# Ighina/MultimodalTopicSegmentation

Measured on AMD Instinct MI355X. Metric: sentences/sec (fwd+bwd), higher is better.
Workload: dtype bf16; 1 GPU; BASELINE configs[1]: restricted-window transformer tagger d=1792 heads=8 ff=256 radius=15 layers=1 focal loss, 64 docs x 256 sentences per GPU, fwd+bwd+Adam(eps 1e-7), inputs resident in HBM; global_batch_docs=64, sentences_per_doc=256, parallelism=dp1 (document-sharded, RCCL all-reduce)

## Files before the change

multimodaltopicsegmentation_amd/csrc/gemm.hip:

```cpp
#include <algorithm>
#include <math.h>
#include <stdlib.h>
#include "common.h"

#include "gemm_common.h"


template <int LAYOUT, typename TC, bool GLDS>
__global__ __launch_bounds__(256, 2) void gemm_bf16_kernel(const GemmArgs a) {
  constexpr bool A_KMAJOR = (LAYOUT == MTS_NT || LAYOUT == MTS_NN);
  constexpr bool B_KMAJOR = (LAYOUT == MTS_NT || LAYOUT == MTS_TT);
  extern __shared__ __attribute__((aligned(16))) char smem[];

  const int tid = threadIdx.x;
  const int lane = tid & 63;
  const int wave = tid >> 6;
  const int wm = wave >> 1, wn = wave & 1;
  const int r16 = lane & 15, g = lane >> 4;

  const int ntn = (a.N + BN - 1) / BN;
  const int ntm = (a.M + BM - 1) / BM;
  const int nt = ntn * ntm;
  int bid = xcd_remap(blockIdx.x, nt);
  const int bm0 = (ntm < ntn ? bid % ntm : bid / ntn) * BM;
// ... 549 lines not shown
    const int e = (int)(i - r * q) * 4;
    float v[4];
    load4<float>(e < D1 ? s1 + r * D1 + e : s2 + r * D2 + (e - D1), v);
    store4<T>(dst + r * D + e, v);
  }
}

extern "C" int mts_cast_concat(void* stream, int dst_dtype, size_t rows, int D1, int D2, const float* src1, const float* src2, void* dst) {
  MTS_CHECK_ARG(src1 && src2 && dst && D1 > 0 && D2 > 0 && D1 % 4 == 0 && D2 % 4 == 0, "mts_cast_concat: bad arguments (widths must be multiples of 4)");
  if (rows == 0) return MTS_OK;
  const int blocks = (int)std::min<size_t>(4096, (rows * ((D1 + D2) / 4) + 255) / 256);
  if (dst_dtype == MTS_BF16) hipLaunchKernelGGL(cast_concat_kernel<bf16_t>, dim3(blocks), dim3(256), 0, (hipStream_t)stream, src1, src2, (bf16_t*)dst, rows, D1, D2);
  else if (dst_dtype == MTS_F32) hipLaunchKernelGGL(cast_concat_kernel<float>, dim3(blocks), dim3(256), 0, (hipStream_t)stream, src1, src2, (float*)dst, rows, D1, D2);
  else { mts_set_error("mts_cast_concat: bad dtype %d", dst_dtype); return MTS_ERR_INVALID; }
  MTS_LAUNCH_CHECK("mts_cast_concat");
  return MTS_OK;
}

extern "C" size_t mts_colsum_workspace(int N) { return (size_t)COLSUM_RS * (size_t)N * sizeof(float); }

extern "C" int mts_colsum(void* stream, int dtype, int M, int N, const void* X, int ldx, float* out, int accumulate,
                          void* partial) {
  MTS_CHECK_ARG(M > 0 && N > 0 && X && out && partial, "mts_colsum: bad arguments");
  MTS_CHECK_ARG(dtype == MTS_F32 || dtype == MTS_BF16, "mts_colsum: bad dtype %d", dtype);
  MTS_CHECK_ARG(ldx % 4 == 0, "mts_colsum: ldx must be a multiple of 4");
  hipStream_t st = (hipStream_t)stream;
  const int nparts = min(COLSUM_RS, M);
  dim3 grid(ceil_div(N, 64), COLSUM_RS);
  (void)nparts;
  if (dtype == MTS_F32)
    hipLaunchKernelGGL(colsum_partial_kernel<float>, grid, dim3(256), 0, st, (const float*)X, M, N, ldx, (float*)partial);
  else
    hipLaunchKernelGGL(colsum_partial_kernel<bf16_t>, grid, dim3(256), 0, st, (const bf16_t*)X, M, N, ldx, (float*)partial);
  hipLaunchKernelGGL(colsum_final_kernel, dim3(ceil_div(N, 64)), dim3(256), 0, st, (const float*)partial, N, COLSUM_RS, out,
                     accumulate);
  MTS_LAUNCH_CHECK("mts_colsum");
  return MTS_OK;
}

extern "C" int mts_cast(void* stream, int dst_dtype, const float* src, void* dst, size_t n) {
  MTS_CHECK_ARG(src && dst, "mts_cast: null pointer");
  if (n == 0) return MTS_OK;
  hipStream_t st = (hipStream_t)stream;
  const int blocks = (int)std::min<size_t>(2048, (n / 4 + 255) / 256 + 1);
  if (dst_dtype == MTS_BF16)
    hipLaunchKernelGGL(cast_kernel<bf16_t>, dim3(blocks), dim3(256), 0, st, src, (bf16_t*)dst, n);
  else if (dst_dtype == MTS_F32)
    hipLaunchKernelGGL(cast_kernel<float>, dim3(blocks), dim3(256), 0, st, src, (float*)dst, n);
  else {
    mts_set_error("mts_cast: bad dtype %d", dst_dtype);
    return MTS_ERR_INVALID;
  }
  MTS_LAUNCH_CHECK("mts_cast");
  return MTS_OK;
}

int mts_launch_gemm256(const GemmArgs& a, int layout, bool c_is_f32, int splits, hipStream_t st);
int mts_launch_gemm224(const GemmArgs& a, int layout, bool c_is_f32, int splits, hipStream_t st);
bool mts_gemm224t_applies(const GemmArgs& a, int layout, bool c_is_f32, int splits);

static thread_local int g_gemm_glds = -1;
static thread_local int g_tile_mode = -1;
static thread_local int g_force_splits = 0;
static thread_local int g_tile_order = 1;
static thread_local int g_gemm_deep = 1;
static thread_local int g_chain = 0;
static thread_local int g_combine = 0;
#define MTS_GEMM_WS_HEAD 8192
static thread_local int g_last_tile = 0, g_last_splits = 0;

static thread_local void (*g_mid_hook)(void) = nullptr;
extern "C" int mts_gemm_set_mid_hook(void (*fn)(void)) { g_mid_hook = fn; return MTS_OK; }

extern "C" int mts_gemm_last_plan(int* tile, int* splits) {
  if (tile) *tile = g_last_tile;
  if (splits) *splits = g_last_splits;
  return MTS_OK;
}

void mts_band_set_mfma(int on);
void mts_band_set_fused(int on);
void mts_full_set_mfma(int on);
void mts_t5_set_mfma(int on);
static thread_local int g_f32_mfma = 1;
static thread_local int g_big_min_k = 256;
static thread_local int g_gemm_variant = 0;
void mts_lstm_pair_set_spin_limit(int n);
void mts_lstm_pair_set_max_pairs(int n);
void mts_lstm_pair_set_parts(int n);
extern "C" int mts_set_option(const char* key, int value) {
  if (!key) return MTS_ERR_INVALID;
  if (!strcmp(key, "gemm_tile")) { g_tile_mode = value; return MTS_OK; }
  if (!strcmp(key, "gemm_glds")) { g_gemm_glds = value; return MTS_OK; }
  if (!strcmp(key, "gemm_splits")) { g_force_splits = value; return MTS_OK; }
  if (!strcmp(key, "gemm_order")) { g_tile_order = value; return MTS_OK; }
  if (!strcmp(key, "gemm_chain")) { g_chain = value; return MTS_OK; }
  if (!strcmp(key, "gemm_combine")) { g_combine = value; return MTS_OK; }
  if (!strcmp(key, "gemm_deep")) { g_gemm_deep = value; return MTS_OK; }
  if (!strcmp(key, "gemm_variant")) { g_gemm_variant = value; return MTS_OK; }
  if (!strcmp(key, "gemm_big_min_k")) { g_big_min_k = value; return MTS_OK; }
  if (!strcmp(key, "gemm_f32_mfma")) { g_f32_mfma = value; return MTS_OK; }
  if (!strcmp(key, "band_mfma")) { mts_band_set_mfma(value); return MTS_OK; }
  if (!strcmp(key, "band_fused_bwd")) { mts_band_set_fused(value); return MTS_OK; }
  if (!strcmp(key, "full_mfma")) { mts_full_set_mfma(value); return MTS_OK; }
  if (!strcmp(key, "t5_mfma")) { mts_t5_set_mfma(value); return MTS_OK; }
  if (!strcmp(key, "lstm_pair_spin_limit")) { mts_lstm_pair_set_spin_limit(value); return MTS_OK; }
  if (!strcmp(key, "lstm_pair_max_pairs")) { mts_lstm_pair_set_max_pairs(value); return MTS_OK; }
  if (!strcmp(key, "lstm_parts")) { mts_lstm_pair_set_parts(value); return MTS_OK; }
  mts_set_error("mts_set_option: unknown key %s", key);
  return MTS_ERR_INVALID;
}

template <int LAYOUT, typename TC>
static void launch_bf16(const GemmArgs& a, int splits, hipStream_t st) {
  const int nt = ceil_div(a.M, BM) * ceil_div(a.N, BN);
  if (g_gemm_glds < 0) {
    const char* e = getenv("MTS_GEMM_GLDS");
    g_gemm_glds = (e && e[0] == '0') ? 0 : 1;
  }
  const bool glds = g_gemm_glds && (a.K % BK == 0) && (a.ksplit % BK == 0) && a.M >= 8 && a.N >= 8;
  if (glds) {
    GemmArgs b = a;
    const bool deep = g_gemm_deep && (size_t)nt * splits <= 256 && a.ksplit >= 4 * BK;
    b.nbuf = deep ? 4 : 2;
    auto k = gemm_bf16_kernel<LAYOUT, TC, true>;
    if (deep && mts_dyn_lds(k, 8 * TILE_BYTES, "gemm") != MTS_OK) b.nbuf = 2;
    hipLaunchKernelGGL(k, dim3(nt, 1, splits), dim3(256), (b.nbuf == 4 ? 8 : 4) * TILE_BYTES, st, b);
  } else {
    hipLaunchKernelGGL((gemm_bf16_kernel<LAYOUT, TC, false>), dim3(nt, 1, splits), dim3(256), 4 * TILE_BYTES, st, a);
  }
}

static void plan_bf16(int c_dtype, int layout, int M, int N, int K, unsigned epilogue, bool has_workspace, size_t workspace_bytes,
                      int* use256_out, int* splits_out) {
  if (g_tile_mode < 0) {
    const char* e = getenv("MTS_GEMM_TILE");
    g_tile_mode = e ? atoi(e) : 0;
  }
  const int tile_mode = g_tile_mode;
  const unsigned plain = epilogue & ~MTS_EPI_ACCUM;
  const bool can_split = (c_dtype == MTS_F32 && plain == 0 && has_workspace && N % 4 == 0 && K >= 2048);
  const bool can256 = (K % BK == 0) && K >= g_big_min_k && M >= 8 && N >= 8 && tile_mode != 128;
  const double bw = 3500.0;
  double best = 1e30;
  int splits = 1;
  int use256 = 0;
  const bool can224 = can256 && (N % 224 == 0) && tile_mode != 256;
  for (int big = 0; big <= (can256 ? 2 : 0); ++big) {
    if (big == 2 && !can224) continue;
    if (tile_mode == 256 && can256 && big != 1) continue;
    if (tile_mode == 224 && can224 && big != 2) continue;
    const int tile = big ? 256 : 128;
    const double slots = big ? 256.0 : 512.0;
    const double t_k = layout == MTS_TN ? (big == 2 ? (M % 256 == 0 ? 0.0160 : 0.0200) : big == 1 ? 0.0218 : 0.0145)
                                        : (big ? 0.0232 * (big == 2 ? 0.875 : 1.0) : 0.0180);
    const double t_0 = big ? 7.7 : 6.5;
    const int nt = ceil_div(M, tile) * (big == 2 ? N / 224 : ceil_div(N, tile));
    for (int sp = 1; sp <= (can_split ? 32 : 1); ++sp) {
      const int ks = ceil_div(ceil_div(K, sp), BK) * BK;
      if (ceil_div(K, ks) != sp) continue;
      if (sp > 1 && (size_t)sp * M * N * sizeof(float) > workspace_bytes) break;
      if (g_force_splits > 0 && can_split && sp != g_force_splits) continue;
      const double rounds = ceil((double)nt * sp / slots);
      const double cost = rounds * (ks * t_k + t_0) + (sp > 1 ? (2.0 * sp + 1.0) * M * N * 4.0 / 1e6 / bw : 0.0);
      if (cost < best) { best = cost; splits = sp; use256 = big; }
    }
  }
  *use256_out = use256;
  *splits_out = splits;
}

int mts_gemm224_last_kernel();
int mts_launch_gemm224t_pair(const GemmArgs& a, int splits, const void* A2, const void* B2, float* slab2, hipStream_t st);
bool mts_gemm224t_applies(const GemmArgs& a, int layout, bool c_is_f32, int splits);

static int wgrad_pair_splits(int M, int N, int K, size_t workspace_bytes) {
  if (M % 256 || N % 224 || K % 64 || K < 256) return -1;
  static int cus = 0;
  if (!cus) { int dev = 0; hipDeviceProp_t pr; cus = (hipGetDevice(&dev) == hipSuccess && hipGetDeviceProperties(&pr, dev) == hipSuccess) ? pr.multiProcessorCount : 256; }
  const int nt = (M / 256) * (N / 224);
  int sp = std::max(1, std::min(32, cus / (2 * nt)));
  for (; sp >= 1; --sp) {
    const int ks = ceil_div(ceil_div(K, sp), BK) * BK;
    if (ceil_div(K, ks) != sp) continue;
    if (ks >= 128 && K - (sp - 1) * ks >= 128 && (size_t)2 * sp * M * N * sizeof(float) <= workspace_bytes) return sp;
  }
  return -1;
}
// ... 158 lines not shown
```

multimodaltopicsegmentation_amd/csrc/norm.hip:

```cpp
#include <algorithm>
#include <type_traits>
#include "common.h"
#include "loss_elems.h"

#define ROW_WAVES 4
#define BWD_MAX_BLOCKS 512

template <typename T, int NV> struct RowRegs {
  float v[NV][4];
  __device__ __forceinline__ void load(const T* row, int D, int lane) {
#pragma unroll
    for (int i = 0; i < NV; ++i) {
      const int e = 4 * (lane + 64 * i);
      if (e < D) load4<T>(row + e, v[i]);
      else { v[i][0] = v[i][1] = v[i][2] = v[i][3] = 0.f; }
    }
  }
  __device__ __forceinline__ void store(T* row, int D, int lane) const {
#pragma unroll
    for (int i = 0; i < NV; ++i) {
      const int e = 4 * (lane + 64 * i);
      if (e < D) store4<T>(row + e, v[i]);
    }
  }
  __device__ __forceinline__ void zero() {
#pragma unroll
    for (int i = 0; i < NV; ++i) v[i][0] = v[i][1] = v[i][2] = v[i][3] = 0.f;
  }
};

template <int NV> __device__ __forceinline__ void row_stats(const float (&x)[NV][4], int D, int lane, float& mean, float& rstd, float eps) {
  float s = 0.f;
#pragma unroll
  for (int i = 0; i < NV; ++i) s += (x[i][0] + x[i][1]) + (x[i][2] + x[i][3]);
  mean = wave_sum(s) / (float)D;
  float q = 0.f;
#pragma unroll
  for (int i = 0; i < NV; ++i) {
    if (4 * (lane + 64 * i) < D) {
#pragma unroll
      for (int j = 0; j < 4; ++j) { const float d = x[i][j] - mean; q += d * d; }
    }
  }
  rstd = 1.0f / sqrtf(wave_sum(q) / (float)D + eps);
}

template <typename T, int NV, int EMBED, bool FULL = false>
__global__ __launch_bounds__(64 * ROW_WAVES) void ln_fwd_kernel(
    const void* __restrict__ xin, const float* __restrict__ pos, int pos_offset, int L, const float* __restrict__ type0,
    const float* __restrict__ gamma, const float* __restrict__ beta, float eps, int rows, int D,
    T* __restrict__ y, T* __restrict__ pre, float* __restrict__ mean_out, float* __restrict__ rstd_out,
    const float* __restrict__ head_w, const float* __restrict__ head_b, int n_out, float* __restrict__ scores,
    const int32_t* __restrict__ row_src, const float* __restrict__ xin2 = nullptr, int D1 = 0) {
  const int lane = threadIdx.x & 63;
  const int row = blockIdx.x * ROW_WAVES + (threadIdx.x >> 6);
  if (row >= rows) return;
  float gv[NV][4], bv[NV][4];
#pragma unroll
  for (int i = 0; i < NV; ++i) {
    const int e = 4 * (lane + 64 * i);
    if (FULL || e < D) { load4<float>(gamma + e, gv[i]); load4<float>(beta + e, bv[i]); }
  }
  float x[NV][4];
  if constexpr (EMBED) {
    const int src = row_src ? row_src[row] : row;
    const int Dx = xin2 ? D1 : D;
    const float* xr = reinterpret_cast<const float*>(xin) + (size_t)src * Dx;
    const float* xr2 = xin2 ? xin2 + (size_t)src * (D - D1) - D1 : xr;
    const float* pr = pos + (size_t)(pos_offset + src % L) * D;
#pragma unroll
    for (int i = 0; i < NV; ++i) {
      const int e = 4 * (lane + 64 * i);
      if (FULL || e < D) {
        float a[4], b[4], c[4];
        if constexpr (EMBED == 2) load4<bf16_t>(reinterpret_cast<const bf16_t*>(xin) + (size_t)src * D + e, a);
        else load4<float>((e < Dx ? xr : xr2) + e, a);
        load4<float>(pr + e, b); load4<float>(type0 + e, c);
#pragma unroll
        for (int j = 0; j < 4; ++j) x[i][j] = (a[j] + b[j]) + c[j];
        if constexpr (sizeof(T) == 2) {
#pragma unroll
          for (int j = 0; j < 4; ++j) x[i][j] = to_f32(from_f32<T>(x[i][j]));
        }
      } else { x[i][0] = x[i][1] = x[i][2] = x[i][3] = 0.f; }
    }
    if (pre) {
#pragma unroll
      for (int i = 0; i < NV; ++i) { const int e = 4 * (lane + 64 * i); if (FULL || e < D) store4<T>(pre + (size_t)row * D + e, x[i]); }
    }
  } else {
    const T* xr = reinterpret_cast<const T*>(xin) + (size_t)row * D;
#pragma unroll
    for (int i = 0; i < NV; ++i) {
      const int e = 4 * (lane + 64 * i);
      if (FULL || e < D) load4<T>(xr + e, x[i]);
      else { x[i][0] = x[i][1] = x[i][2] = x[i][3] = 0.f; }
    }
  }
  float mean, rstd;
  row_stats<NV>(x, D, lane, mean, rstd, eps);
  float hs[4] = {0.f, 0.f, 0.f, 0.f};
  const float* hwp = head_w ? head_w : gamma;
  const int hw_max = head_w ? n_out - 1 : 0;
#pragma unroll
  for (int i = 0; i < NV; ++i) {
    const int e = 4 * (lane + 64 * i);
    if (FULL || e < D) {
#pragma unroll
      for (int j = 0; j < 4; ++j) x[i][j] = (x[i][j] - mean) * rstd * gv[i][j] + bv[i][j];
      if (head_w) {
#pragma unroll
        for (int c = 0; c < 4; ++c) {
          float w[4];
          load4<float>(hwp + (size_t)min(c, hw_max) * D + e, w);
#pragma unroll
          for (int j = 0; j < 4; ++j) hs[c] += to_f32(from_f32<T>(x[i][j])) * w[j];
        }
      }
    }
  }
  if (y) {
#pragma unroll
    for (int i = 0; i < NV; ++i) {
      const int e = 4 * (lane + 64 * i);
      if (FULL || e < D) store4<T>(y + (size_t)row * D + e, x[i]);
    }
  }
  if (lane == 0 && mean_out) { mean_out[row] = mean; rstd_out[row] = rstd; }
  if (head_w) {
    for (int c = 0; c < n_out; ++c) {
      const float s = wave_sum(hs[c]);
      if (lane == 0) scores[(size_t)row * n_out + c] = s + head_b[c];
    }
  }
}

template <typename T>
__global__ __launch_bounds__(64 * ROW_WAVES) void head_fwd_kernel(const T* __restrict__ x, int ldx, int rows, int D, int n_out,
                                                                const float* __restrict__ w, const float* __restrict__ b,
                                                                float* __restrict__ scores) {
  const int lane = threadIdx.x & 63;
  const int row = blockIdx.x * ROW_WAVES + (threadIdx.x >> 6);
  if (row >= rows) return;
  float hs[4] = {0.f, 0.f, 0.f, 0.f};
  for (int e = 4 * lane; e < D; e += 256) {
    float xv[4];
    load4<T>(x + (size_t)row * ldx + e, xv);
    for (int c = 0; c < n_out; ++c) {
      float wv[4];
      load4<float>(w + (size_t)c * D + e, wv);
#pragma unroll
      for (int j = 0; j < 4; ++j) hs[c] += xv[j] * wv[j];
    }
  }
  for (int c = 0; c < n_out; ++c) {
    const float s = wave_sum(hs[c]);
    if (lane == 0) scores[(size_t)row * n_out + c] = s + b[c];
  }
}

template <typename T>
__global__ __launch_bounds__(256) void head_bwd_data_kernel(const float* __restrict__ ds, const float* __restrict__ w, int rows, int D,
                                                            int n_out, T* __restrict__ dx, int lddx, int accumulate) {
  const size_t idx = (size_t)blockIdx.x * 256 + threadIdx.x;
  const int per_row = D / 4;
  const size_t total = (size_t)rows * per_row;
  if (idx >= total) return;
  const int row = (int)(idx / per_row);
  const int e = 4 * (int)(idx % per_row);
  float o[4] = {0.f, 0.f, 0.f, 0.f};
  if (accumulate) load4<T>(dx + (size_t)row * lddx + e, o);
  for (int c = 0; c < n_out; ++c) {
    const float s = ds[(size_t)row * n_out + c];
    float wv[4];
    load4<float>(w + (size_t)c * D + e, wv);
#pragma unroll
    for (int j = 0; j < 4; ++j) o[j] += s * wv[j];
  }
  store4<T>(dx + (size_t)row * lddx + e, o);
}

struct EmbArgs { int B, L, Bc, nchunks; const int32_t* row0; const int32_t* lengths; float* dpos_part; };

template <typename T, int NV, bool WIDE, bool FULL = false, int NHG = 0, bool EMB = false>
__global__ __launch_bounds__(64 * ROW_WAVES, 2) void ln_bwd_kernel(
    const T* __restrict__ x, const T* __restrict__ dy_, const float* __restrict__ dlogit, const float* __restrict__ head_w, int n_out,
    const float* __restrict__ gamma, const float* __restrict__ mean, const float* __restrict__ rstd, int rows, int D,
    T* __restrict__ dx, float* __restrict__ partial, const EmbArgs ea) {
  static_assert(!(EMB && (WIDE || NHG > 0)), "the embedding form has no head and D <= 2048");
  constexpr bool HG = NHG > 0;
  constexpr int NR = HG ? NHG + 1 : EMB ? 2 : 3;
  constexpr int NS = HG ? NHG + 2 : NR;
  constexpr int NA = HG ? NHG : 2;
  const T* __restrict__ dy = HG ? nullptr : dy_;
  __shared__ float red[ROW_WAVES][NR][64 * 4];
  __shared__ __attribute__((aligned(16))) float gam_s[NV * 256];
  __shared__ __attribute__((aligned(16))) float hw_s[EMB ? 1 : 4][EMB ? 4 : NV * 256];
  __shared__ __attribute__((aligned(16))) float task_s[EMB ? ROW_WAVES : 1][EMB ? NV * 256 : 4];
  const int lane = threadIdx.x & 63;
  const int wave = __builtin_amdgcn_readfirstlane(threadIdx.x >> 6);
  const int col0 = WIDE ? (int)blockIdx.y * (NV * 256) : 0;
  for (int idx = threadIdx.x; idx < NV * 256; idx += 64 * ROW_WAVES) {
    const int e = col0 + idx;
    gam_s[idx] = (e < D) ? gamma[e] : 0.f;
    if constexpr (!EMB) {
      if (head_w)
        for (int c = 0; c < n_out; ++c) hw_s[c][idx] = (e < D) ? head_w[(size_t)c * D + e] : 0.f;
    }
  }
  __syncthreads();
  float acc[NA][NV][4];
  float dxs[NV][4];
  float tsum[HG ? NHG : 1];
#pragma unroll
  for (int i = 0; i < NV; ++i)
#pragma unroll
    for (int j = 0; j < 4; ++j) {
// ... 685 lines not shown
    else { const float tv[4] = {t.x, t.y, t.z, t.w}; for (int j = 0; j < 4 && e + j < len; ++j) o[e + j] = tv[j]; }
  }
}

int mts_slab_reduce_rows(hipStream_t st, const float* partial, int nblocks, int D, float* out) {
  SlabOuts so = {{out, nullptr, nullptr, nullptr, nullptr, nullptr}, -1, 0, nullptr, -1, 0};
  hipLaunchKernelGGL(slab_reduce_kernel, dim3(ceil_div(D, SR_COLS), 1), dim3(256), 0, st, partial, nblocks, 1, D, so);
  MTS_LAUNCH_CHECK("slab_reduce");
  return MTS_OK;
}

template <typename T>
__global__ __launch_bounds__(256) void embed_bwd_kernel(const T* __restrict__ dpre, int B, int L, int D, float* __restrict__ dpos, int pos_offset,
                                                        const int32_t* __restrict__ row0, const int32_t* __restrict__ lengths) {
  const size_t idx = (size_t)blockIdx.x * 256 + threadIdx.x;
  const int per_row = D / 4;
  if (idx >= (size_t)L * per_row) return;
  const int i = (int)(idx / per_row), e = 4 * (int)(idx % per_row);
  float s[4] = {0.f, 0.f, 0.f, 0.f};
  int b = 0;
  if (row0) {
    for (; b < B; ++b) {
      if (i < lengths[b]) {
        float v[4];
        load4<T>(dpre + ((size_t)row0[b] + i) * D + e, v);
#pragma unroll
        for (int j = 0; j < 4; ++j) s[j] += v[j];
      }
    }
  }
  for (; b + 7 < B; b += 8) {
    float v[8][4];
#pragma unroll
    for (int u = 0; u < 8; ++u) load4<T>(dpre + ((size_t)(b + u) * L + i) * D + e, v[u]);
#pragma unroll
    for (int u = 0; u < 8; ++u)
#pragma unroll
      for (int j = 0; j < 4; ++j) s[j] += v[u][j];
  }
  for (; b < B; ++b) {
    float v[4];
    load4<T>(dpre + ((size_t)b * L + i) * D + e, v);
#pragma unroll
    for (int j = 0; j < 4; ++j) s[j] += v[j];
  }
  float* o = dpos + (size_t)(pos_offset + i) * D + e;
  float cur[4];
  load4<float>(o, cur);
#pragma unroll
  for (int j = 0; j < 4; ++j) cur[j] += s[j];
  store4<float>(o, cur);
}
static inline int pick_nv(int D) {
  const int need = ceil_div(D, 256);
  if (need <= 1) return 1;
  if (need <= 2) return 2;
  if (need <= 4) return 4;
  if (need == 7) return 7;
  if (need <= 8) return 8;
  if (need <= 16) return 16;
  return 0;
}

template <typename F> static inline void dispatch_nv(int nv, F&& f) {
  switch (nv) {
    case 1: f(std::integral_constant<int, 1>{}); break;
    case 2: f(std::integral_constant<int, 2>{}); break;
    case 4: f(std::integral_constant<int, 4>{}); break;
    case 7: f(std::integral_constant<int, 7>{}); break;
    case 8: f(std::integral_constant<int, 8>{}); break;
    default: f(std::integral_constant<int, 16>{}); break;
  }
}
template <typename F> static inline void dispatch_nv8(int nv, F&& f) {
  switch (nv) {
    case 1: f(std::integral_constant<int, 1>{}); break;
    case 2: f(std::integral_constant<int, 2>{}); break;
    case 4: f(std::integral_constant<int, 4>{}); break;
    case 7: f(std::integral_constant<int, 7>{}); break;
    default: f(std::integral_constant<int, 8>{}); break;
  }
}

template <typename T, int EMBED>
static int ln_fwd_launch(hipStream_t st, const void* x, const float* pos, int pos_offset, int L, const float* type0, const float* gamma,
                         const float* beta, float eps, int rows, int D, void* y, void* pre, float* mean, float* rstd,
                         const float* head_w, const float* head_b, int n_out, float* scores, const int32_t* row_src = nullptr,
                         const float* x2 = nullptr, int D1 = 0) {
  const int nv = pick_nv(D);
  MTS_UNSUPPORTED(nv > 0 && D % 4 == 0, "layernorm: D=%d must be a multiple of 4 and <= 4096", D);
  dim3 grid(ceil_div(rows, ROW_WAVES)), block(64 * ROW_WAVES);
  dispatch_nv(nv, [&](auto nvc) {
    constexpr int NV = decltype(nvc)::value;
    if (D == NV * 256)
      hipLaunchKernelGGL((ln_fwd_kernel<T, NV, EMBED, true>), grid, block, 0, st, x, pos, pos_offset, L, type0, gamma, beta, eps, rows, D, (T*)y,
                         (T*)pre, mean, rstd, head_w, head_b, n_out, scores, row_src, x2, D1);
    else
      hipLaunchKernelGGL((ln_fwd_kernel<T, NV, EMBED>), grid, block, 0, st, x, pos, pos_offset, L, type0, gamma, beta, eps, rows, D, (T*)y,
                         (T*)pre, mean, rstd, head_w, head_b, n_out, scores, row_src, x2, D1);
  });
  MTS_LAUNCH_CHECK("layernorm_fwd");
  return MTS_OK;
}

static int embed_ln_fwd(void* stream, int dtype, int B, int L, int D, const float* x, const float* x2, int D1, const float* pos, int pos_offset,
                        const float* type0, const float* gamma, const float* beta, float eps, void* y, void* pre, float* mean, float* rstd,
                        const int32_t* row_src, int n_rows, const char* who) {
  MTS_CHECK_ARG(B > 0 && L > 0 && D > 0 && x && pos && type0 && gamma && beta && y, "%s: bad arguments", who);
  MTS_CHECK_ARG(!row_src || (n_rows > 0 && n_rows <= B * L), "%s: packed form needs 0 < n_rows <= B*L", who);
  MTS_CHECK_ARG(!x2 || (D1 > 0 && D1 < D && D1 % 4 == 0), "%s: the first part's width must be a multiple of 4 inside (0, D)", who);
  const int rows = row_src ? n_rows : B * L;
  if (dtype == MTS_F32)
    return ln_fwd_launch<float, 1>((hipStream_t)stream, x, pos, pos_offset, L, type0, gamma, beta, eps, rows, D, y, pre, mean, rstd,
                                      nullptr, nullptr, 0, nullptr, row_src, x2, D1);
  if (dtype == MTS_BF16)
    return ln_fwd_launch<bf16_t, 1>((hipStream_t)stream, x, pos, pos_offset, L, type0, gamma, beta, eps, rows, D, y, pre, mean, rstd,
                                       nullptr, nullptr, 0, nullptr, row_src, x2, D1);
  mts_set_error("%s: bad dtype %d", who, dtype);
  return MTS_ERR_INVALID;
}

extern "C" int mts_embed_layernorm_fwd(void* stream, int dtype, int B, int L, int D, const float* x, const float* pos, int pos_offset,
                                       const float* type0, const float* gamma, const float* beta, float eps, void* y, void* pre,
                                       float* mean, float* rstd, const int32_t* row_src, int n_rows) {
  return embed_ln_fwd(stream, dtype, B, L, D, x, nullptr, 0, pos, pos_offset, type0, gamma, beta, eps, y, pre, mean, rstd, row_src, n_rows,
                      "mts_embed_layernorm_fwd");
}

extern "C" int mts_embed_layernorm_fwd_x16(void* stream, int B, int L, int D, const void* x_bf16, const float* pos, int pos_offset, const float* type0,
                                           const float* gamma, const float* beta, float eps, void* y, void* pre, float* mean, float* rstd,
                                           const int32_t* row_src, int n_rows) {
  MTS_CHECK_ARG(B > 0 && L > 0 && D > 0 && x_bf16 && pos && type0 && gamma && beta && y, "mts_embed_layernorm_fwd_x16: bad arguments");
  MTS_CHECK_ARG(!row_src || (n_rows > 0 && n_rows <= B * L), "mts_embed_layernorm_fwd_x16: packed form needs 0 < n_rows <= B*L");
  MTS_CHECK_ARG(((uintptr_t)x_bf16 & 7) == 0, "mts_embed_layernorm_fwd_x16: x must be 8-byte aligned");
  const int rows = row_src ? n_rows : B * L;
  return ln_fwd_launch<bf16_t, 2>((hipStream_t)stream, x_bf16, pos, pos_offset, L, type0, gamma, beta, eps, rows, D, y, pre, mean, rstd, nullptr, nullptr, 0,
                                  nullptr, row_src, nullptr, 0);
}

extern "C" int mts_embed_layernorm_fwd2(void* stream, int dtype, int B, int L, int D1, int D2, const float* x1, const float* x2, const float* pos,
                                        int pos_offset, const float* type0, const float* gamma, const float* beta, float eps, void* y, void* pre,
                                        float* mean, float* rstd, const int32_t* row_src, int n_rows) {
  MTS_CHECK_ARG(x2 && D2 > 0 && D2 % 4 == 0, "mts_embed_layernorm_fwd2: second part missing or its width not a multiple of 4");
  return embed_ln_fwd(stream, dtype, B, L, D1 + D2, x1, x2, D1, pos, pos_offset, type0, gamma, beta, eps, y, pre, mean, rstd, row_src, n_rows,
                      "mts_embed_layernorm_fwd2");
}

extern "C" int mts_layernorm_fwd(void* stream, int dtype, int rows, int D, const void* x, const float* gamma, const float* beta, float eps,
                                 void* y, float* mean, float* rstd, const float* head_w, const float* head_b, int n_out, float* scores) {
  MTS_CHECK_ARG(rows > 0 && D > 0 && x && gamma && beta && (y || (head_w && mean && rstd)), "mts_layernorm_fwd: bad arguments (y may be NULL only with a fused head and saved statistics)");
  MTS_CHECK_ARG(!head_w || (head_b && scores && n_out >= 1 && n_out <= 4), "mts_layernorm_fwd: fused head needs head_b, scores, n_out<=4");
  if (dtype == MTS_F32)
    return ln_fwd_launch<float, 0>((hipStream_t)stream, x, nullptr, 0, 1, nullptr, gamma, beta, eps, rows, D, y, nullptr, mean, rstd,
                                       head_w, head_b, n_out, scores);
  if (dtype == MTS_BF16)
    return ln_fwd_launch<bf16_t, 0>((hipStream_t)stream, x, nullptr, 0, 1, nullptr, gamma, beta, eps, rows, D, y, nullptr, mean, rstd,
                                        head_w, head_b, n_out, scores);
  mts_set_error("mts_layernorm_fwd: bad dtype %d", dtype);
  return MTS_ERR_INVALID;
}

extern "C" size_t mts_layernorm_bwd_workspace(int D) { return (size_t)BWD_MAX_BLOCKS * 6 * (size_t)D * sizeof(float); }

template <typename T>
static int ln_bwd_launch(hipStream_t st, int rows, int D, const void* x, const void* dy, const float* dlogit, const float* head_w, int n_out,
                         const float* gamma, const float* beta, const float* mean, const float* rstd, void* dx, float* dgamma, float* dbeta,
                         float* dxsum, float* dhead_w, float* dhead_b, void* partial) {
  const int nv = pick_nv(D);
  MTS_UNSUPPORTED(nv > 0 && D % 4 == 0, "layernorm_bwd: D=%d must be a multiple of 4 and <= 4096", D);
  const int blocks = std::min(BWD_MAX_BLOCKS, ceil_div(rows, ROW_WAVES));
  const int nhg = dhead_w ? n_out : 0;
  const EmbArgs ea = {0, 0, 0, 0, nullptr, nullptr, nullptr};
  auto go = [&](auto k, dim3 grid) {
// ... 17 lines not shown
    if (nhg == 1) go(ln_bwd_kernel<T, 8, true, false, 1>, dim3(blocks, ceil_div(D, 2048)));
    else if (nhg == 2) go(ln_bwd_kernel<T, 8, true, false, 2>, dim3(blocks, ceil_div(D, 2048)));
    else go(ln_bwd_kernel<T, 8, true>, dim3(blocks, ceil_div(D, 2048)));
  }
  if (nhg == 1)
    hipLaunchKernelGGL(ln_head_final_kernel<1>, dim3(ceil_div(D, 32)), dim3(256), 0, st, (const float*)partial, blocks, D, head_w, gamma, beta, dgamma,
                       dbeta, dxsum, dhead_w, dhead_b, (const float*)nullptr, (float*)nullptr);
  else if (nhg == 2)
    hipLaunchKernelGGL(ln_head_final_kernel<2>, dim3(ceil_div(D, 32)), dim3(256), 0, st, (const float*)partial, blocks, D, head_w, gamma, beta, dgamma,
                       dbeta, dxsum, dhead_w, dhead_b, (const float*)nullptr, (float*)nullptr);
  else {
    SlabOuts so = {{dgamma, dbeta, dxsum, nullptr, nullptr, nullptr}, -1, 0, nullptr, -1, 0};
    hipLaunchKernelGGL(slab_reduce_kernel, dim3(ceil_div(D, SR_COLS), 3), dim3(256), 0, st, (const float*)partial, blocks, 3, D, so);
  }
  MTS_LAUNCH_CHECK("layernorm_bwd");
  return MTS_OK;
}

extern "C" int mts_layernorm_bwd(void* stream, int dtype, int rows, int D, const void* x, const void* dy, const float* dlogit,
                                 const float* head_w, int n_out, const float* gamma, const float* mean, const float* rstd, void* dx,
                                 float* dgamma, float* dbeta, float* dxsum, void* partial, const float* beta, float* dhead_w, float* dhead_b) {
  MTS_CHECK_ARG(rows > 0 && D > 0 && x && gamma && mean && rstd && dx && partial, "mts_layernorm_bwd: bad arguments");
  MTS_CHECK_ARG(dy || head_w, "mts_layernorm_bwd: needs dy and/or a fused head gradient");
  MTS_CHECK_ARG(!head_w || (dlogit && n_out >= 1 && n_out <= 4), "mts_layernorm_bwd: fused head needs dlogit, n_out<=4");
  MTS_CHECK_ARG(!dhead_w || (head_w && beta && dhead_b && n_out <= 2 && !dy),
                "mts_layernorm_bwd: head parameter gradients need head_w, beta, dhead_b, n_out <= 2 and dy == NULL (the last layer)");
  if (dtype == MTS_F32)
    return ln_bwd_launch<float>((hipStream_t)stream, rows, D, x, dy, dlogit, head_w, n_out, gamma, beta, mean, rstd, dx, dgamma, dbeta, dxsum, dhead_w, dhead_b, partial);
  if (dtype == MTS_BF16)
    return ln_bwd_launch<bf16_t>((hipStream_t)stream, rows, D, x, dy, dlogit, head_w, n_out, gamma, beta, mean, rstd, dx, dgamma, dbeta, dxsum, dhead_w, dhead_b, partial);
  mts_set_error("mts_layernorm_bwd: bad dtype %d", dtype);
  return MTS_ERR_INVALID;
}

extern "C" int mts_layernorm_loss_tail_supported(int dtype, int D, int n_out) {
  return (dtype == MTS_F32 || dtype == MTS_BF16) && (n_out == 1 || n_out == 2) && D % 256 == 0 &&
         (D == 256 || D == 512 || D == 1024 || D == 1792 || D == 2048);
}

template <typename T>
static int ln_tail_launch(hipStream_t st, int rows, int D, const void* x, const float* gamma, const float* beta, float eps, const float* head_w,
                          const float* head_b, int n_out, void* dx, float* dgamma, float* dbeta, float* dxsum, float* dhead_w, float* dhead_b,
                          float* ws, const TailArgs& ta0) {
  const int nv = D / 256;
  const int blocks = std::min(BWD_MAX_BLOCKS, ceil_div(rows, ROW_WAVES));
  TailArgs ta = ta0;
  ta.loss_part = ws + (size_t)BWD_MAX_BLOCKS * 5 * D;
  dispatch_nv8(nv, [&](auto nvc) {
    constexpr int NV = decltype(nvc)::value;
    if (n_out == 1)
      hipLaunchKernelGGL((ln_tail_kernel<T, NV, 1>), dim3(blocks), dim3(64 * ROW_WAVES), 0, st, (const T*)x, gamma, beta, eps, head_w, head_b, rows, D, (T*)dx, ws, ta);
    else
      hipLaunchKernelGGL((ln_tail_kernel<T, NV, 2>), dim3(blocks), dim3(64 * ROW_WAVES), 0, st, (const T*)x, gamma, beta, eps, head_w, head_b, rows, D, (T*)dx, ws, ta);
  });
  const dim3 fgrid(ceil_div(D, 32));
  if (n_out == 1)
    hipLaunchKernelGGL(ln_head_final_kernel<1>, fgrid, dim3(256), 0, st, (const float*)ws, blocks, D, head_w, gamma, beta, dgamma, dbeta, dxsum, dhead_w, dhead_b,
                       (const float*)ta.loss_part, ta.loss_out);
  else
    hipLaunchKernelGGL(ln_head_final_kernel<2>, fgrid, dim3(256), 0, st, (const float*)ws, blocks, D, head_w, gamma, beta, dgamma, dbeta, dxsum, dhead_w, dhead_b,
                       (const float*)ta.loss_part, ta.loss_out);
  MTS_LAUNCH_CHECK("mts_layernorm_loss_tail");
  return MTS_OK;
}

extern "C" int mts_layernorm_loss_tail(void* stream, int dtype, int rows, int D, const void* x, const float* gamma, const float* beta, float eps,
                                       const float* head_w, const float* head_b, int n_out, int loss_kind, int B, int L, int Lt, const float* targets,
                                       const int32_t* lengths, float alpha, float gamma_focal, float grad_scale, const int32_t* row_src, int n_rows,
                                       float* scores, float* loss_out, void* dx, float* dgamma, float* dbeta, float* dxsum, float* dhead_w,
                                       float* dhead_b, void* workspace) {
  MTS_CHECK_ARG(rows > 0 && D > 0 && x && gamma && beta && head_w && head_b && targets && scores && loss_out && dx && dgamma && dbeta && dhead_w &&
                dhead_b && workspace, "mts_layernorm_loss_tail: bad arguments");
  MTS_CHECK_ARG(B > 0 && L > 0 && Lt >= L, "mts_layernorm_loss_tail: bad batch shape");
  MTS_CHECK_ARG(loss_kind == MTS_LOSS_CE || loss_kind == MTS_LOSS_BCE || loss_kind == MTS_LOSS_FOCAL, "Choose one of CrossEntropy or BinaryCrossEntropy as loss function");
  MTS_CHECK_ARG((loss_kind == MTS_LOSS_CE) ? n_out == 2 : n_out == 1, "mts_layernorm_loss_tail: n_out=%d does not match the loss kind", n_out);
  MTS_CHECK_ARG(row_src ? (n_rows == rows && rows <= B * L) : rows == B * L, "mts_layernorm_loss_tail: rows must be B*L, or n_rows of a packed batch");
  MTS_UNSUPPORTED(mts_layernorm_loss_tail_supported(dtype, D, n_out), "mts_layernorm_loss_tail: D=%d / n_out=%d not covered (see mts_layernorm_loss_tail_supported)", D, n_out);
  const TailArgs ta = {loss_kind, B, L, Lt, n_rows, targets, lengths, row_src, alpha, gamma_focal, grad_scale, scores, nullptr, loss_out};
  if (dtype == MTS_F32)
    return ln_tail_launch<float>((hipStream_t)stream, rows, D, x, gamma, beta, eps, head_w, head_b, n_out, dx, dgamma, dbeta, dxsum, dhead_w, dhead_b, (float*)workspace, ta);
  return ln_tail_launch<bf16_t>((hipStream_t)stream, rows, D, x, gamma, beta, eps, head_w, head_b, n_out, dx, dgamma, dbeta, dxsum, dhead_w, dhead_b, (float*)workspace, ta);
}

static inline int emb_chunks(int B, int L) { return std::max(1, std::min(B, ceil_div(4 * BWD_MAX_BLOCKS, L))); }
extern "C" size_t mts_embed_layernorm_bwd_workspace(int B, int L, int D) {
  return ((size_t)BWD_MAX_BLOCKS * 2 + POS_SPLIT + (size_t)emb_chunks(B, L) * L) * (size_t)D * sizeof(float);
}

template <typename T>
static int emb_bwd_launch(hipStream_t st, int B, int L, int D, const void* pre, const void* dh, const float* gamma, const float* mean, const float* rstd,
                          float* dgamma, float* dbeta, float* dtype0, float* dpos, int pos_offset, const int32_t* row0, const int32_t* lengths,
                          int n_rows, float* ws) {
  const int nv = pick_nv(D);
  MTS_UNSUPPORTED(nv > 0 && nv <= 8 && D % 4 == 0, "embed_layernorm_bwd: D=%d must be a multiple of 4 and <= 2048", D);
  const int C = emb_chunks(B, L), Bc = ceil_div(B, C);
  const int nchunks = ceil_div(B, Bc);
  const int ntasks = L * nchunks;
  const int blocks = std::min(BWD_MAX_BLOCKS, ceil_div(ntasks, ROW_WAVES));
  float* slabs = ws;
  float* tpart = ws + (size_t)BWD_MAX_BLOCKS * 2 * D;
  float* part = tpart + (size_t)POS_SPLIT * D;
  float* out_rows = dpos + (size_t)pos_offset * D;
  EmbArgs ea = {B, L, Bc, nchunks, row0, lengths, part};
  if (row0) {
    hipError_t e = hipMemsetAsync(part, 0, (size_t)nchunks * L * D * sizeof(float), st);
    if (e != hipSuccess) { mts_set_error("embed_layernorm_bwd: hipMemsetAsync: %s", hipGetErrorString(e)); return MTS_ERR_LAUNCH; }
  }
  dispatch_nv8(nv, [&](auto nvc) {
    constexpr int NV = decltype(nvc)::value;
    if (D == NV * 256)
      hipLaunchKernelGGL((ln_bwd_kernel<T, NV, false, true, 0, true>), dim3(blocks), dim3(64 * ROW_WAVES), 0, st, (const T*)pre, (const T*)dh,
                         (const float*)nullptr, (const float*)nullptr, 0, gamma, mean, rstd, n_rows, D, (T*)nullptr, slabs, ea);
    else
      hipLaunchKernelGGL((ln_bwd_kernel<T, NV, false, false, 0, true>), dim3(blocks), dim3(64 * ROW_WAVES), 0, st, (const T*)pre, (const T*)dh,
                         (const float*)nullptr, (const float*)nullptr, 0, gamma, mean, rstd, n_rows, D, (T*)nullptr, slabs, ea);
  });
  const int ysplit = std::max(1, std::min(POS_SPLIT, L / 32));
  hipLaunchKernelGGL(pos_sum_kernel, dim3(ceil_div(D, 32), ysplit), dim3(256), 0, st, (const float*)part, nchunks, L, D, out_rows, tpart);
  SlabOuts so = {{dgamma, dbeta, dtype0, nullptr, nullptr, nullptr}, -1, 0, tpart, 2, ysplit};
  hipLaunchKernelGGL(slab_reduce_kernel, dim3(ceil_div(D, SR_COLS), 3), dim3(256), 0, st, (const float*)slabs, blocks, 2, D, so);
  MTS_LAUNCH_CHECK("embed_layernorm_bwd");
  return MTS_OK;
}

extern "C" int mts_embed_layernorm_bwd(void* stream, int dtype, int B, int L, int D, const void* pre, const void* dh, const float* gamma,
                                       const float* mean, const float* rstd, float* dgamma, float* dbeta, float* dtype0, float* dpos,
                                       int pos_offset, const int32_t* row0, const int32_t* lengths, int n_rows, void* workspace, size_t workspace_bytes) {
  MTS_CHECK_ARG(B > 0 && L > 0 && D > 0 && pre && dh && gamma && mean && rstd && dgamma && dbeta && dtype0 && dpos && workspace,
                "mts_embed_layernorm_bwd: bad arguments");
  MTS_CHECK_ARG(!row0 || (lengths && n_rows > 0 && n_rows <= B * L), "mts_embed_layernorm_bwd: packed form needs lengths and 0 < n_rows <= B*L");
  if (workspace_bytes < mts_embed_layernorm_bwd_workspace(B, L, D)) { mts_set_error("mts_embed_layernorm_bwd: workspace too small"); return MTS_ERR_WORKSPACE; }
  const int rows = row0 ? n_rows : B * L;
  if (dtype == MTS_F32)
    return emb_bwd_launch<float>((hipStream_t)stream, B, L, D, pre, dh, gamma, mean, rstd, dgamma, dbeta, dtype0, dpos, pos_offset, row0, lengths, rows, (float*)workspace);
  if (dtype == MTS_BF16)
    return emb_bwd_launch<bf16_t>((hipStream_t)stream, B, L, D, pre, dh, gamma, mean, rstd, dgamma, dbeta, dtype0, dpos, pos_offset, row0, lengths, rows, (float*)workspace);
  mts_set_error("mts_embed_layernorm_bwd: bad dtype %d", dtype);
  return MTS_ERR_INVALID;
}

extern "C" int mts_embed_bwd(void* stream, int dtype, int B, int L, int D, const void* dpre, float* dpos, int pos_offset, const int32_t* row0,
                             const int32_t* lengths) {
  MTS_CHECK_ARG(B > 0 && L > 0 && D > 0 && D % 4 == 0 && dpre && dpos, "mts_embed_bwd: bad arguments");
  MTS_CHECK_ARG(!row0 || lengths, "mts_embed_bwd: packed form needs lengths");
  hipStream_t st = (hipStream_t)stream;
  const int blocks = (int)(((size_t)L * (D / 4) + 255) / 256);
  if (dtype == MTS_F32) hipLaunchKernelGGL(embed_bwd_kernel<float>, dim3(blocks), dim3(256), 0, st, (const float*)dpre, B, L, D, dpos, pos_offset, row0, lengths);
  else if (dtype == MTS_BF16) hipLaunchKernelGGL(embed_bwd_kernel<bf16_t>, dim3(blocks), dim3(256), 0, st, (const bf16_t*)dpre, B, L, D, dpos, pos_offset, row0, lengths);
  else { mts_set_error("mts_embed_bwd: bad dtype %d", dtype); return MTS_ERR_INVALID; }
  MTS_LAUNCH_CHECK("mts_embed_bwd");
  return MTS_OK;
}

extern "C" int mts_head_fwd(void* stream, int dtype, int rows, int D, int n_out, const void* x, int ldx, const float* w, const float* b,
                            float* scores) {
  MTS_CHECK_ARG(rows > 0 && D > 0 && D % 4 == 0 && ldx % 4 == 0 && n_out >= 1 && n_out <= 4 && x && w && b && scores, "mts_head_fwd: bad arguments");
  hipStream_t st = (hipStream_t)stream;
  dim3 grid(ceil_div(rows, ROW_WAVES)), block(64 * ROW_WAVES);
  if (dtype == MTS_F32) hipLaunchKernelGGL(head_fwd_kernel<float>, grid, block, 0, st, (const float*)x, ldx, rows, D, n_out, w, b, scores);
  else if (dtype == MTS_BF16) hipLaunchKernelGGL(head_fwd_kernel<bf16_t>, grid, block, 0, st, (const bf16_t*)x, ldx, rows, D, n_out, w, b, scores);
  else { mts_set_error("mts_head_fwd: bad dtype %d", dtype); return MTS_ERR_INVALID; }
  MTS_LAUNCH_CHECK("mts_head_fwd");
  return MTS_OK;
}

extern "C" int mts_head_bwd_params(void* stream, int dtype, int rows, int D, int n_out, const void* x, int ldx, const float* dscores,
                                   float* dw, float* db, void* partial) {
// ... 92 lines not shown
```

Baseline: 9.505 million sentences/s.

## Add persistent streaming embed-layernorm forward kernel with row prefetch

Adds a persistent grid-stride kernel for the embedding+layernorm forward. Each wave walks several documents at the same sentence position, reuses the positional row, and prefetches the next row's inputs while normalising the current one. Gamma, beta and type vectors are staged in shared memory once per block. The kernel is enabled by default through a new option and aims to cut memory latency stalls and redundant parameter loads, at the cost of more register pressure and a fixed grid sized from the CU count.

Measured after the change: 9.558 million sentences/s, median of 6. About the same (+0.6%).

```diff
diff --git a/multimodaltopicsegmentation_amd/csrc/gemm.hip b/multimodaltopicsegmentation_amd/csrc/gemm.hip
--- a/multimodaltopicsegmentation_amd/csrc/gemm.hip
+++ b/multimodaltopicsegmentation_amd/csrc/gemm.hip
@@ -655,6 +655,7 @@
 void mts_band_set_fused(int on);
 void mts_full_set_mfma(int on);
 void mts_t5_set_mfma(int on);
+void mts_norm_set_embed_fwd_stream(int v);
 static thread_local int g_f32_mfma = 1;
 static thread_local int g_big_min_k = 256;
 static thread_local int g_gemm_variant = 0;
@@ -677,6 +678,7 @@
   if (!strcmp(key, "band_fused_bwd")) { mts_band_set_fused(value); return MTS_OK; }
   if (!strcmp(key, "full_mfma")) { mts_full_set_mfma(value); return MTS_OK; }
   if (!strcmp(key, "t5_mfma")) { mts_t5_set_mfma(value); return MTS_OK; }
+  if (!strcmp(key, "embed_fwd_stream")) { mts_norm_set_embed_fwd_stream(value); return MTS_OK; }
   if (!strcmp(key, "lstm_pair_spin_limit")) { mts_lstm_pair_set_spin_limit(value); return MTS_OK; }
   if (!strcmp(key, "lstm_pair_max_pairs")) { mts_lstm_pair_set_max_pairs(value); return MTS_OK; }
   if (!strcmp(key, "lstm_parts")) { mts_lstm_pair_set_parts(value); return MTS_OK; }
diff --git a/multimodaltopicsegmentation_amd/csrc/norm.hip b/multimodaltopicsegmentation_amd/csrc/norm.hip
--- a/multimodaltopicsegmentation_amd/csrc/norm.hip
+++ b/multimodaltopicsegmentation_amd/csrc/norm.hip
@@ -1,4 +1,5 @@
 #include <algorithm>
+#include <atomic>
 #include <type_traits>
 #include "common.h"
 #include "loss_elems.h"
@@ -133,6 +134,118 @@
       if (lane == 0) scores[(size_t)row * n_out + c] = s + head_b[c];
     }
   }
+}
+
+template <typename T, int NV, int EMBED, bool PRE>
+__global__ __launch_bounds__(64 * ROW_WAVES, 2) void embed_fwd_stream_kernel(
+    const void* __restrict__ xin, const float* __restrict__ xin2, int D1, const float* __restrict__ pos, const float* __restrict__ type0,
+    const float* __restrict__ gamma, const float* __restrict__ beta, float eps, int B, int L, int Bc, int nchunks,
+    T* __restrict__ y, T* __restrict__ pre, float* __restrict__ mean_out, float* __restrict__ rstd_out) {
+  static_assert(EMBED == 1 || EMBED == 2, "the embedding block only");
+  constexpr int D = NV * 256;
+  using TX = std::conditional_t<EMBED == 2, bf16_t, float>;
+  __shared__ __attribute__((aligned(16))) float gam_s[D], bet_s[D], typ_s[D];
+  const int lane = threadIdx.x & 63;
+  const int wave = __builtin_amdgcn_readfirstlane(threadIdx.x >> 6);
+  const int stride = gridDim.x * ROW_WAVES, ntasks = L * nchunks;
+  int task = min((int)blockIdx.x * ROW_WAVES + wave, ntasks - 1);
+  const int Dx = xin2 ? D1 : D;
+  Pack<TX, 4> px[NV];
+  typedef float f32x4 __attribute__((ext_vector_type(4)));
+  f32x4 pp[NV];
+  auto fetch_x = [&](int r) {
+    const TX* xr = reinterpret_cast<const TX*>(xin) + (size_t)r * Dx;
+    const TX* xr2 = xr;
+    if constexpr (EMBED == 1) { if (xin2) xr2 = xin2 + (size_t)r * (D - D1) - D1; }
+#pragma unroll
+    for (int i = 0; i < NV; ++i) {
+      const int e = 4 * (lane + 64 * i);
+      px[i].load((e < Dx ? xr : xr2) + e);
+    }
+  };
+  auto fetch_pos = [&](int i_) {
+#pragma unroll
+    for (int i = 0; i < NV; ++i) pp[i] = *reinterpret_cast<const f32x4*>(pos + (size_t)i_ * D + 4 * (lane + 64 * i));
+  };
+  int ti = 0, tb = 0, tbend = 0;
+  auto open_task = [&](int t) {
+    ti = __builtin_amdgcn_readfirstlane(t % L);
+    tb = __builtin_amdgcn_readfirstlane(t / L) * Bc;
+    tbend = min(B, tb + Bc);
+  };
+  auto do_row = [&](int row) {
+    float x[NV][4];
+#pragma unroll
+    for (int i = 0; i < NV; ++i) {
+      asm volatile("" : "+v"(pp[i]));
+      const float4 c = *reinterpret_cast<const float4*>(typ_s + 4 * (lane + 64 * i));
+      const float cv[4] = {c.x, c.y, c.z, c.w};
+#pragma unroll
+      for (int j = 0; j < 4; ++j) {
+        x[i][j] = (px[i].get(j) + pp[i][j]) + cv[j];
+        if constexpr (sizeof(T) == 2) x[i][j] = to_f32(from_f32<T>(x[i][j]));
+        asm volatile("" : "+v"(x[i][j]));
+      }
+    }
+    __builtin_amdgcn_sched_barrier(0);
+    int nrow = -1, npos = -1;
+    if (tb + 1 < tbend) {
+      ++tb;
+      nrow = tb * L + ti;
+    } else {
+      task += stride;
+      if (task < ntasks) {
+        open_task(task);
+        nrow = tb * L + ti;
+        npos = ti;
+      }
+    }
+    if (nrow >= 0) fetch_x(nrow);
+    if (npos >= 0) fetch_pos(npos);
+    __builtin_amdgcn_sched_barrier(0);
+    if constexpr (PRE) {
+#pragma unroll
+      for (int i = 0; i < NV; ++i) store4<T>(pre + (size_t)row * D + 4 * (lane + 64 * i), x[i]);
+    }
+    float mean, rstd;
+    row_stats<NV>(x, D, lane, mean, rstd, eps);
+#pragma unroll
+    for (int i = 0; i < NV; ++i) {
+      const float4 g = *reinterpret_cast<const float4*>(gam_s + 4 * (lane + 64 * i));
+      const float4 b = *reinterpret_cast<const float4*>(bet_s + 4 * (lane + 64 * i));
+      const float gv[4] = {g.x, g.y, g.z, g.w}, bv[4] = {b.x, b.y, b.z, b.w};
+#pragma unroll
+      for (int j = 0; j < 4; ++j) x[i][j] = (x[i][j] - mean) * rstd * gv[j] + bv[j];
+      store4<T>(y + (size_t)row * D + 4 * (lane + 64 * i), x[i]);
+    }
+    if (lane == 0 && mean_out) { mean_out[row] = mean; rstd_out[row] = rstd; }
+    return nrow;
+  };
+  open_task(task);
+  int row = tb * L + ti;
+  fetch_x(row);
+  fetch_pos(ti);
+  {
+    constexpr int NK = (NV + ROW_WAVES - 1) / ROW_WAVES;
+    float4 par[NK][3];
+#pragma unroll
+    for (int k = 0; k < NK; ++k) {
+      const int e = 4 * (lane + 64 * min(wave + ROW_WAVES * k, NV - 1));
+      par[k][0] = *reinterpret_cast<const float4*>(gamma + e);
+      par[k][1] = *reinterpret_cast<const float4*>(beta + e);
+      par[k][2] = *reinterpret_cast<const float4*>(type0 + e);
+    }
+#pragma unroll
+    for (int k = 0; k < NK; ++k) {
+      const int e = 4 * (lane + 64 * min(wave + ROW_WAVES * k, NV - 1));
+      *reinterpret_cast<float4*>(gam_s + e) = par[k][0];
+      *reinterpret_cast<float4*>(bet_s + e) = par[k][1];
+      *reinterpret_cast<float4*>(typ_s + e) = par[k][2];
+    }
+  }
+  __syncthreads();
+  row = do_row(row);
+  while (row >= 0) row = do_row(row);
 }
 
 template <typename T>
@@ -984,6 +1097,34 @@
   }
 }
 
+static inline int emb_chunks(int B, int L, int waves = ROW_WAVES * BWD_MAX_BLOCKS) { return std::max(1, std::min(B, ceil_div(waves, L))); }
+
+static thread_local int g_embed_fwd_stream = 1;
+void mts_norm_set_embed_fwd_stream(int v) { g_embed_fwd_stream = v; }
+#define EMBED_STREAM_RESIDENT 2
+
+template <typename T, int NV, int EMBED>
+static void embed_fwd_stream_launch(hipStream_t st, const void* x, const float* x2, int D1, const float* pos_rows, const float* type0, const float* gamma,
+                                    const float* beta, float eps, int B, int L, T* y, T* pre, float* mean, float* rstd) {
+  static std::atomic<int> ncu{0};
+  if (!ncu) {
+    int dev = 0, n = 0;
+    if (hipGetDevice(&dev) != hipSuccess || hipDeviceGetAttribute(&n, hipDeviceAttributeMultiprocessorCount, dev) != hipSuccess || n <= 0) n = 256;
+    ncu = n;
+  }
+  int max_blocks = EMBED_STREAM_RESIDENT * (int)ncu;
+  if (g_embed_fwd_stream > 1) max_blocks = std::min(max_blocks, g_embed_fwd_stream);
+  const int Bc = ceil_div(B, emb_chunks(B, L, ROW_WAVES * max_blocks));
+  const int nchunks = ceil_div(B, Bc);
+  const int blocks = (int)std::min<long long>(max_blocks, ceil_div((long long)L * nchunks, (long long)ROW_WAVES));
+  if (pre)
+    hipLaunchKernelGGL((embed_fwd_stream_kernel<T, NV, EMBED, true>), dim3(blocks), dim3(64 * ROW_WAVES), 0, st, x, x2, D1, pos_rows, type0, gamma, beta, eps,
+                       B, L, Bc, nchunks, y, pre, mean, rstd);
+  else
+    hipLaunchKernelGGL((embed_fwd_stream_kernel<T, NV, EMBED, false>), dim3(blocks), dim3(64 * ROW_WAVES), 0, st, x, x2, D1, pos_rows, type0, gamma, beta, eps,
+                       B, L, Bc, nchunks, y, pre, mean, rstd);
+}
+
 template <typename T, int EMBED>
 static int ln_fwd_launch(hipStream_t st, const void* x, const float* pos, int pos_offset, int L, const float* type0, const float* gamma,
                          const float* beta, float eps, int rows, int D, void* y, void* pre, float* mean, float* rstd,
@@ -991,6 +1132,16 @@
                          const float* x2 = nullptr, int D1 = 0) {
   const int nv = pick_nv(D);
   MTS_UNSUPPORTED(nv > 0 && D % 4 == 0, "layernorm: D=%d must be a multiple of 4 and <= 4096", D);
+  if constexpr (EMBED != 0) {
+    if (g_embed_fwd_stream && D == nv * 256 && nv <= 8 && !row_src && !head_w) {
+      dispatch_nv8(nv, [&](auto nvc) {
+        constexpr int NV = decltype(nvc)::value;
+        embed_fwd_stream_launch<T, NV, EMBED>(st, x, x2, D1, pos + (size_t)pos_offset * D, type0, gamma, beta, eps, rows / L, L, (T*)y, (T*)pre, mean, rstd);
+      });
+      MTS_LAUNCH_CHECK("embed_layernorm_fwd");
+      return MTS_OK;
+    }
+  }
   dim3 grid(ceil_div(rows, ROW_WAVES)), block(64 * ROW_WAVES);
   dispatch_nv(nv, [&](auto nvc) {
     constexpr int NV = decltype(nvc)::value;
@@ -1174,7 +1325,6 @@
   return ln_tail_launch<bf16_t>((hipStream_t)stream, rows, D, x, gamma, beta, eps, head_w, head_b, n_out, dx, dgamma, dbeta, dxsum, dhead_w, dhead_b, (float*)workspace, ta);
 }
 
-static inline int emb_chunks(int B, int L) { return std::max(1, std::min(B, ceil_div(4 * BWD_MAX_BLOCKS, L))); }
 extern "C" size_t mts_embed_layernorm_bwd_workspace(int B, int L, int D) {
   return ((size_t)BWD_MAX_BLOCKS * 2 + POS_SPLIT + (size_t)emb_chunks(B, L) * L) * (size_t)D * sizeof(float);
 }
```
